# vqdang/hover_net

Measured on AMD Instinct MI355X. Metric: tiles/sec (270x270, batch 32) end-to-end incl. watershed, higher is better.
Workload: dtype fp32

## Files before the change

hover_net_amd/csrc/hvn_api.hip:

```cpp
#include <hip/hip_runtime.h>
#include <stdio.h>
#include <string.h>

#include <vector>

#include "../../include/hvn.h"
#include "hvn_kernels.h"

static thread_local char g_err[512] = "";

static int fail(int code, const char *fmt, const char *a = "", long b = 0)
{
    snprintf(g_err, sizeof(g_err), fmt, a, b);
    return code;
}

extern "C" {

int hvn_version(void) { return 104; }

#ifndef HVN_BUILD_ID
#define HVN_BUILD_ID "unstamped"
#endif
static const char hvn_build_tag[] = "hvn-build-id:" HVN_BUILD_ID;
// ... 48 lines not shown

int hvn_profile_conv_ms_list(double *out, int cap)
{
    if (g_ev_used < 2) return 0;
    hipEventSynchronize(g_ev[g_ev_used - 1]);
    int n = 0;
    for (size_t i = 0; i + 1 < g_ev_used && n < cap; i += 2, ++n) {
        float ms = 0.f;
        hipEventElapsedTime(&ms, g_ev[i], g_ev[i + 1]);
        out[n] = ms;
    }
    return n;
}

static bool aligned16(const void *p) { return (((uintptr_t)p) & 15) == 0; }

static int run_one(const hvn_op *op, int batch, hipStream_t s)
{
    switch (op->kind) {
    case HVN_OP_CONV0: {
        Conv0Args a;
        a.img = op->x.base;
        a.isn = op->x.sn; a.isy = op->x.sy; a.isx = op->x.sx; a.isc = op->x.sc ? op->x.sc : 1;
        a.is_f32 = op->x_dtype;
        a.H = op->x.h; a.W = op->x.w;
        a.w = op->w; a.bias = op->bias;
        a.y = (float *)op->y.base;
        a.ysn = op->y.sn; a.ysy = op->y.sy; a.ysx = op->y.sx;
        a.N = batch; a.Ho = op->y.h; a.Wo = op->y.w; a.pad = op->pad_t; a.relu = op->relu; a.out_bf16 = op->act_dtype == 1;
        if (op->kh != 7 || op->kw != 7 || op->x.c != 3 || op->y.c != 64 || !op->w || !op->bias)
            return fail(HVN_E_ARG, "conv0: expects 7x7x3->64 with bias%s", "");
        if (!aligned16(a.y) || (a.ysx & 3) || (a.ysy & 3) || (a.ysn & 3)) return fail(HVN_E_ARG, "conv0: output view not 16-byte aligned%s", "");
        return hvn_launch_conv0(a, s);
    }
    case HVN_OP_CONV: {
        ConvArgs a;
        memset(&a, 0, sizeof(a));
        a.x = (const float *)op->x.base;
        a.xsn = op->x.sn; a.xsy = op->x.sy; a.xsx = op->x.sx;
        a.H = op->x.h; a.W = op->x.w; a.Cin = op->x.c;
        a.w = op->w; a.bias = op->bias;
        a.pre_s = op->pre_scale; a.pre_b = op->pre_shift;
        a.post_s = op->post_scale; a.post_b = op->post_shift;
        a.res = (const float *)op->res.base;
        a.rsn = op->res.sn; a.rsy = op->res.sy; a.rsx = op->res.sx;
        a.y = (float *)op->y.base;
        a.ysn = op->y.sn; a.ysy = op->y.sy; a.ysx = op->y.sx;
        a.N = batch; a.Ho = op->y.h; a.Wo = op->y.w; a.Cout = op->cout;
        a.KH = op->kh; a.KW = op->kw; a.stride = op->stride; a.pad_t = op->pad_t; a.pad_l = op->pad_l;
        a.relu = op->relu;
        a.groups = op->groups > 1 ? op->groups : 1;
        a.x2 = (const float *)op->x2.base;
        a.x2sn = op->x2.sn; a.x2sy = op->x2.sy; a.x2sx = op->x2.sx;
        a.Cin2 = a.x2 ? op->x2.c : 0;
        a.stride2 = op->_rsv > 0 ? op->_rsv : 1;
        if (a.x2 && (op->kh != 1 || op->kw != 1 || a.stride != 1 || a.Cin2 % 32 || !aligned16(a.x2) || ((a.x2sn | a.x2sy | a.x2sx) & 3) ||
                     a.pre_s || (long)(a.Ho - 1) * a.stride2 >= op->x2.h || (long)(a.Wo - 1) * a.stride2 >= op->x2.w))
            return fail(HVN_E_ARG, "conv: second input needs a 1x1 stride-1 op without prologue and a view that covers the output grid%s", "");
        a.M = (long)batch * a.Ho * a.Wo;
        if (!a.x || !a.w || !a.y) return fail(HVN_E_ARG, "conv: null pointer%s", "");
        if (a.Cin % 32) return fail(HVN_E_ARG, "conv: input channels must be a multiple of 32 (got %s%ld)", "", a.Cin);
        if (!aligned16(a.x) || !aligned16(a.w) || (a.xsx & 3) || (a.xsy & 3) || (a.xsn & 3))
            return fail(HVN_E_ARG, "conv: input view / weights not 16-byte aligned%s", "");
        if ((a.pre_s && !aligned16(a.pre_s)) || (a.pre_b && !aligned16(a.pre_b)) || (!a.pre_s != !a.pre_b))
            return fail(HVN_E_ARG, "conv: prologue vectors must be 16-byte aligned and come in pairs%s", "");
        if (!a.post_s != !a.post_b) return fail(HVN_E_ARG, "conv: epilogue affine must come in pairs%s", "");
        if (op->y.c != op->cout) return fail(HVN_E_ARG, "conv: output view channels != cout%s", "");
        a.nbatch = op->nbatch > 1 ? op->nbatch : 1;
        a.xb = op->batch_stride[0]; a.wb = op->batch_stride[1]; a.yb = op->batch_stride[2];
        if (a.nbatch > 1 && ((a.xb | a.wb | a.yb) & 3)) return fail(HVN_E_ARG, "conv: batch strides must keep 16-byte alignment%s", "");
        const bool bf16 = op->act_dtype == 1;
        if (bf16 && (((a.xsx | a.xsy | a.xsn) & 7) || (a.x2 && ((a.x2sx | a.x2sy | a.x2sn) & 7)) || a.nbatch > 1))
            return fail(HVN_E_ARG, "conv(bf16): input strides must be multiples of 8 elements; no batched launch%s", "");
        if (g_prof) prof_mark(s);
        const bool x3 = op->act_dtype == 2 || op->act_dtype == 3;
        if (x3 && (a.groups > 1 || (a.nbatch > 1 && (a.wb & 7)))) return fail(HVN_E_ARG, "conv(bf16x3): no grouped convs; batch stride of the planes must keep 16-byte alignment%s", "");
        int rc;
        if (bf16 && (op->tile_n == 896 || op->tile_n == 640))
            rc = hvn_launch_conv_bf16g(a, op->tile_n == 896 ? 256 : 128, s);
        else if (bf16)
            rc = hvn_launch_conv_bf16(a, op->tile_n, s);
        else if (x3 && (op->tile_n == 896 || op->tile_n == 640))
            rc = hvn_launch_conv_x3g(a, op->tile_n == 896 ? 256 : 128, op->act_dtype == 3 ? 6 : 9, s);
        else
            rc = x3 ? hvn_launch_conv_x3(a, op->tile_n, op->act_dtype == 3 ? 6 : 9, s) : hvn_launch_conv(a, op->tile_n, s);
        if (g_prof) prof_mark(s);
        if (rc) return fail(rc == -1 ? HVN_E_ARG : HVN_E_LAUNCH, "conv: launch failed (tile_n=%s%ld)", "", op->tile_n);
        return 0;
    }
    case HVN_OP_CHAIN: {
        ChainArgs a;
        memset(&a, 0, sizeof(a));
        a.x = (const float *)op->x.base;
        a.xsn = op->x.sn; a.xsy = op->x.sy; a.xsx = op->x.sx; a.K1 = op->x.c;
        a.x2 = (const float *)op->x2.base;
        a.x2sn = op->x2.sn; a.x2sy = op->x2.sy; a.x2sx = op->x2.sx;
        a.K1b = a.x2 ? op->x2.c : 0;
        a.stride2 = op->_rsv > 0 ? op->_rsv : 1;
        a.w1 = op->w;
        a.res = (const float *)op->res.base;
        a.rsn = op->res.sn; a.rsy = op->res.sy; a.rsx = op->res.sx;
        a.y = (float *)op->y.base;
        a.ysn = op->y.sn; a.ysy = op->y.sy; a.ysx = op->y.sx; a.C = op->cout;
        a.post_s = op->post_scale; a.post_b = op->post_shift;
        a.pre_s = op->pre_scale; a.pre_b = op->pre_shift;
        a.w2 = op->w2; a.bias2 = op->bias2; a.relu2 = 1;
        a.y2 = (float *)op->y2.base;
        a.y2sn = op->y2.sn; a.y2sy = op->y2.sy; a.y2sx = op->y2.sx; a.N2 = op->cout2;
        a.N = batch; a.Ho = op->y.h; a.Wo = op->y.w;
        a.M = (long)batch * a.Ho * a.Wo;
        a.bm = op->tile_n == 64 ? 64 : 128;
        const bool cx3 = op->act_dtype == 2 || op->act_dtype == 3;
        const bool cbf = op->act_dtype == 1;
        if (op->act_dtype != 0 && !cx3 && !cbf) return fail(HVN_E_ARG, "chain: act_dtype 0 (fp32), 1 (bf16) or 2 | 3 (fp32 with bf16x3 products)%s", "");
        if (cbf) {
            if (!a.x || !a.w1 || !a.y || !a.w2 || !a.y2) return fail(HVN_E_ARG, "chain: null pointer%s", "");
            if (op->kh != 1 || op->kw != 1 || op->stride != 1 || op->pad_t || op->pad_l || op->relu || op->bias)
                return fail(HVN_E_ARG, "chain: the first conv is a plain 1x1 (no bias / relu of its own)%s", "");
            if (!hvn_chain_bf16_supported(a.K1, a.K1b, a.C, a.N2) || op->y.c != a.C || op->y2.c != a.N2)
                return fail(HVN_E_ARG, "chain (bf16): needs input channels in slabs of 64 (64 or 128 in all), cout %% 256 == 0, cout2 in {64, 128} (cout2 = %s%ld)", "", a.N2);
            if (op->x.h != a.Ho || op->x.w != a.Wo || op->y2.h != a.Ho || op->y2.w != a.Wo ||
                (a.x2 && ((long)(a.Ho - 1) * a.stride2 >= op->x2.h || (long)(a.Wo - 1) * a.stride2 >= op->x2.w)))
                return fail(HVN_E_ARG, "chain: views do not cover the output grid%s", "");
            if (a.res && (a.rsn != a.ysn || a.rsy != a.ysy || a.rsx != a.ysx || op->res.c != a.C))
                return fail(HVN_E_ARG, "chain: the residual view must have the output's strides%s", "");
            if (!aligned16(a.x) || !aligned16(a.w1) || !aligned16(a.w2) || !aligned16(a.y) || !aligned16(a.y2) || (a.res && !aligned16(a.res)) ||
                (a.x2 && !aligned16(a.x2)) || ((a.xsn | a.xsy | a.xsx | a.ysn | a.ysy | a.ysx | a.y2sn | a.y2sy | a.y2sx | a.x2sn | a.x2sy | a.x2sx) & 7))
                return fail(HVN_E_ARG, "chain (bf16): views / weights not 16-byte aligned%s", "");
            if ((!a.pre_s != !a.pre_b) || (!a.post_s != !a.post_b) || (a.pre_s && (!aligned16(a.pre_s) || !aligned16(a.pre_b))) ||
                (a.post_s && (!aligned16(a.post_s) || !aligned16(a.post_b))) || (a.bias2 && !aligned16(a.bias2)))
                return fail(HVN_E_ARG, "chain: per-channel vectors must be 16-byte aligned and come in pairs%s", "");
            if (g_prof) prof_mark(s);
            const int rcb = hvn_launch_conv_chain_bf16(a, s);
            if (g_prof) prof_mark(s);
            if (rcb) return fail(rcb == -1 ? HVN_E_ARG : HVN_E_LAUNCH, "chain (bf16): launch failed (cout2=%s%ld)", "", a.N2);
            return 0;
        }
        if (!a.x || !a.w1 || !a.y || !a.w2 || !a.y2) return fail(HVN_E_ARG, "chain: null pointer%s", "");
        if (op->kh != 1 || op->kw != 1 || op->stride != 1 || op->pad_t || op->pad_l || op->relu || op->bias)
            return fail(HVN_E_ARG, "chain: the first conv is a plain 1x1 (no bias / relu of its own)%s", "");
        if (!hvn_chain_supported(a.C, a.N2) || op->y.c != a.C || op->y2.c != a.N2 || a.K1 % 32 || a.K1b % 32 || a.K1 + a.K1b < 64)
            return fail(HVN_E_ARG, "chain: needs cout %% 64 == 0, cout2 in {64, 128}, input channels in slabs of 32 (>= 64) (cout2 = %s%ld)", "", a.N2);
        if (op->x.h != a.Ho || op->x.w != a.Wo || op->y2.h != a.Ho || op->y2.w != a.Wo ||
            (a.x2 && ((long)(a.Ho - 1) * a.stride2 >= op->x2.h || (long)(a.Wo - 1) * a.stride2 >= op->x2.w)))
            return fail(HVN_E_ARG, "chain: views do not cover the output grid%s", "");
        if (a.res && (a.rsn != a.ysn || a.rsy != a.ysy || a.rsx != a.ysx || op->res.c != a.C))
            return fail(HVN_E_ARG, "chain: the residual view must have the output's strides%s", "");
        if (!aligned16(a.x) || !aligned16(a.w1) || !aligned16(a.w2) || !aligned16(a.y) || !aligned16(a.y2) || (a.res && !aligned16(a.res)) ||
            (a.x2 && !aligned16(a.x2)) || ((a.xsn | a.xsy | a.xsx | a.ysn | a.ysy | a.ysx | a.y2sn | a.y2sy | a.y2sx | a.x2sn | a.x2sy | a.x2sx) & 3))
            return fail(HVN_E_ARG, "chain: views / weights not 16-byte aligned%s", "");
        if ((!a.pre_s != !a.pre_b) || (!a.post_s != !a.post_b) || (a.pre_s && (!aligned16(a.pre_s) || !aligned16(a.pre_b))) ||
            (a.post_s && (!aligned16(a.post_s) || !aligned16(a.post_b))) || (a.bias2 && !aligned16(a.bias2)))
            return fail(HVN_E_ARG, "chain: per-channel vectors must be 16-byte aligned and come in pairs%s", "");
        if (g_prof) prof_mark(s);
        int rc;
        if (cx3 && op->tile_n == 1152)
            rc = hvn_launch_conv_chain_x3r(a, op->act_dtype == 3 ? 6 : 9, s);
        else
            rc = cx3 ? hvn_launch_conv_chain_x3(a, op->act_dtype == 3 ? 6 : 9, s) : hvn_launch_conv_chain(a, s);
        if (g_prof) prof_mark(s);
        if (rc) return fail(rc == -1 ? HVN_E_ARG : HVN_E_LAUNCH, "chain: launch failed (cout2=%s%ld)", "", a.N2);
        return 0;
    }
    case HVN_OP_WINO_IN:
    case HVN_OP_WINO_OUT: {
        WinoArgs a;
// ... 118 lines not shown
```

hover_net_amd/csrc/hvn_kernels.h:

```cpp
#pragma once
#include <hip/hip_runtime.h>
#include <stdint.h>

#include <atomic>

static inline int hvn_max_lds_once(const void *kern, int bytes, std::atomic<unsigned long long> &done)
{
    int dev = 0;
    if (hipGetDevice(&dev) != hipSuccess) return -2;
    const unsigned long long bit = 1ull << (dev & 63);
    if (done.load(std::memory_order_acquire) & bit) return 0;
    if (hipFuncSetAttribute(kern, hipFuncAttributeMaxDynamicSharedMemorySize, bytes) != hipSuccess) return -2;
    done.fetch_or(bit, std::memory_order_release);
    return 0;
}

struct ConvArgs {
    const float *x;
    long xsn, xsy, xsx;
    int H, W, Cin;
    const float *w;
    const float *bias, *pre_s, *pre_b, *post_s, *post_b;
    const float *res;
    long rsn, rsy, rsx;
    float *y;
    long ysn, ysy, ysx;
    int N, Ho, Wo, Cout, KH, KW, stride, pad_t, pad_l, relu;
    long M;
    long m_tiles;
    int n_tiles;
    int groups;
    const float *x2;
    long x2sn, x2sy, x2sx;
    int Cin2, stride2;
    int nbatch;
    unsigned long long *dbg;
    long xb, wb, yb;
};

int hvn_launch_conv(const ConvArgs &a, int tile_n, hipStream_t stream);

#ifndef HVN_CONV_XCD_CONTIG
#define HVN_CONV_XCD_CONTIG 1
#endif
static __device__ __forceinline__ int hvn_m_tile(int xcd, int seq_m, int groups, bool contiguous)
{
    return (HVN_CONV_XCD_CONTIG && contiguous) ? xcd * groups + seq_m : seq_m * 8 + xcd;
}

struct ChainArgs {
    const float *x;
    long xsn, xsy, xsx;
    int K1;
    const float *x2;
    long x2sn, x2sy, x2sx;
    int K1b, stride2;
    const float *w1;
    const float *res;
    long rsn, rsy, rsx;
    float *y;
    long ysn, ysy, ysx;
    int C;
    const float *post_s, *post_b, *pre_s, *pre_b;
    const float *w2;
    const float *bias2;
    int relu2;
    float *y2;
    long y2sn, y2sy, y2sx;
    int N2;
    int N, Ho, Wo;
    long M;
    int bm;
    unsigned long long *dbg;
};
int hvn_launch_conv_chain(const ChainArgs &a, hipStream_t stream);
int hvn_chain_supported(int c, int n2);
int hvn_chain_bf16_supported(int k1, int k1b, int c, int n2);
int hvn_launch_conv_chain_bf16(const ChainArgs &a, hipStream_t stream);
int hvn_launch_conv_chain_x3(const ChainArgs &a, int terms, hipStream_t stream);
int hvn_chain_x3r_supported(const ChainArgs &a);
int hvn_launch_conv_chain_x3r(const ChainArgs &a, int terms, hipStream_t stream);
int hvn_launch_conv_bf16(const ConvArgs &a, int tile_n, hipStream_t stream);
int hvn_launch_conv_bf16g(const ConvArgs &a, int bm, hipStream_t stream);
int hvn_launch_conv_x3(const ConvArgs &a, int tile_n, int terms, hipStream_t stream);
int hvn_launch_conv_x3g(const ConvArgs &a, int bm, int terms, hipStream_t stream);
int hvn_conv_x3g_supported(const ConvArgs &a, int bm);
int hvn_launch_split_x3(const float *src, uint16_t *dst, long granules, hipStream_t stream);

struct Conv0Args {
    const void *img;
    long isn, isy, isx, isc;
    int is_f32;
    int H, W;
    const float *w;
    const float *bias;
    float *y;
    long ysn, ysy, ysx;
    int N, Ho, Wo, pad;
    int relu;
    int out_bf16;
};
int hvn_launch_conv0(const Conv0Args &a, hipStream_t stream);

struct UpAddArgs {
    const float *lo;
    long lsn, lsy, lsx;
    const float *skip;
    long ssn, ssy, ssx;
    float *y;
    long ysn, ysy, ysx;
    int N, H, W, C;
    int bf16;
};
int hvn_launch_upadd(const UpAddArgs &a, hipStream_t stream);

struct HeadArgs {
    const float *x;
    long xsn, xsy, xsx;
    const float *w;
    const float *bias;
    float *y;
    int N, H, W, Cout;
    int in_bf16;
};
int hvn_launch_head(const HeadArgs &a, hipStream_t stream);

int hvn_launch_extract_patches(const uint8_t *img, int H, int W, const int32_t *coords, int P, int win, int pad_t, int pad_l, uint8_t *out,
                               hipStream_t stream);

struct PredMapArgs {
    const float *tp, *np, *hv;
    float *y;
    int N, H, W, nr_types;
};
int hvn_launch_predmap(const PredMapArgs &a, hipStream_t stream);

struct WinoArgs {
    const float *x;
    long xsn, xsy, xsx;
    float *y;
    long ysn, ysy, ysx;
    const float *mat;
    const float *bias;
    int N, H, W, C;
    int ty, tx, pad, relu;
    int m;
    int r;
    int accum;
    const float *lo;
    long lsn, lsy, lsx;
};
int hvn_launch_wino_in(const WinoArgs &a, hipStream_t stream);
int hvn_launch_wino_out(const WinoArgs &a, hipStream_t stream);

struct PackArgs {
    const float *src;
    float *dst;
    int cout, cin_g, groups, taps;
    int mode;
    int lead_pad;
    const float *gmat;
};
int hvn_launch_pack_w(const PackArgs &a, hipStream_t stream);
int hvn_launch_pack_w_multi(const PackArgs *tbl, const int *first_block, int n, long blocks, hipStream_t stream);

struct WgradArgs {
    const float *x;
    long xsn, xsy, xsx;
    int H, W, Cin;
// ... 114 lines not shown
```

hover_net_amd/engine.py:

```python
import ctypes

import numpy as np
import torch

from . import lib as L
from . import plan as PL


def _view_struct(v, base_ptr, sn, itemsize=4):
    b = v.buf
    sx = b.c
    sy = b.w * b.c
    s = L.hvn_view()
    s.base = base_ptr + (v.y0 * sy + v.x0 * sx + v.c0) * itemsize
    s.sn, s.sy, s.sx = sn, sy, sx
    s.h, s.w, s.c, s.sc = v.h, v.w, v.c, 1
    return s


WG_SLOTS = 512
WG_SLOTS_NARROW = 768
NARROW_TILE_COST = 0.45


def pick_tile_n(op, batch):
    import math
    import os

    if op.tile_n != 128 or os.environ.get("HVN_TILE_SELECT", "auto") == "0":
        return op.tile_n
    force = os.environ.get("HVN_FORCE_TILE_N")
    if force:
        return int(force)
    slots64 = int(os.environ.get("HVN_WG_SLOTS_64", WG_SLOTS_NARROW))
    cost64 = float(os.environ.get("HVN_NARROW_COST", NARROW_TILE_COST))
    m_tiles = math.ceil(batch * op.y.h * op.y.w / 128.0)
    nb = int(op.extra.get("nbatch", 1))
    wide = math.ceil(m_tiles * math.ceil(op.cout / 128.0) * nb / WG_SLOTS)
    narrow = math.ceil(m_tiles * math.ceil(op.cout / 64.0) * nb / slots64) * cost64
    return 64 if narrow < wide else 128


_STREAM_POOL, _STREAM_CHOICE = {}, {}


def lane_stream_pool(device, count):
    have = _STREAM_POOL.setdefault(str(device), [])
    while len(have) < count:
        have.append(torch.cuda.Stream(device))
    return have


_TILE_CACHE = {}
X3G_256, X3G_128 = 128 + 0x300, 128 + 0x200
X3R = 128 + 0x400


def x3g_forms_for(op):
    import os

    want = os.environ.get("HVN_X3G", "1")
    if want == "0" or op.cout < 128 or int(op.extra.get("groups", 1)) != 1:
        return ()
    cin = op.x.c
    forms = []
    for code, bm, na in ((X3G_256, 256, 3), (X3G_128, 128, 2)):
        if want not in ("1", str(code)):
            continue
        if op.pre is not None and bm == 256 and na * bm * 128 + 2 * 3 * 128 * 64 + 2 * cin * 4 > 160 * 1024:
            continue
        forms.append(code)
    return tuple(forms)


def to_bf16_bits(a):
    u = np.ascontiguousarray(a, np.float32).view(np.uint32)
    return ((u + (((u >> 16) & 1) + 0x7FFF)) >> 16).astype(np.uint16)


def repack_conv_bf16(w32):
    cp, s32, taps, _ = w32.shape
    if s32 % 2:
        w32 = np.concatenate([w32, np.zeros((cp, 1, taps, 32), np.float32)], 1)
        s32 += 1
    w = w32.reshape(cp, s32 // 2, 2, taps, 32).transpose(0, 1, 3, 2, 4).reshape(cp, s32 // 2, taps, 64)
    return to_bf16_bits(w)


def split_bf16x3(w32):
    w = np.ascontiguousarray(w32, np.float32)

    def bf(a):
        bits = to_bf16_bits(a)
        return bits, (bits.astype(np.uint32) << 16).view(np.float32)

    h, hf = bf(w)
    r = w - hf
    m, mf = bf(r)
    l, _ = bf(r - mf)
    return h, m, l


def pack_conv_x3(w32):
    lead = w32.shape[:-3]
    kt = w32.shape[-3] * w32.shape[-2]
    planes = split_bf16x3(w32.reshape(lead + (kt, 32)))
    return np.stack(planes, axis=-2)


def pack_conv_x3_device(w32, device):
    w = torch.from_numpy(np.ascontiguousarray(w32, np.float32).reshape(-1, 32)).to(device)
    h = w.to(torch.bfloat16)
    r = w - h.float()
    m = r.to(torch.bfloat16)
    l = (r - m.float()).to(torch.bfloat16)
    return torch.stack((h, m, l), dim=1).view(torch.int16).reshape(-1)


class Engine:
    def __init__(self, plan, max_batch=32, device="cuda", n_split=None, dtype="fp32", n_lanes=None):
        L.require_gpu()
        assert dtype in ("fp32", "bf16")
        self.dtype = dtype
        self.isz = 4 if dtype == "fp32" else 2
        if dtype == "bf16" and any(op.kind in (PL.OP_WINO_IN, PL.OP_WINO_OUT) for op in plan.ops):
            raise ValueError("the bf16 path runs direct convolutions: build the plan with winograd=0")
        self.plan = plan
        self.max_batch = int(max_batch)
        self.device = torch.device(device)
        import os
        dflt = ("2", "2") if dtype == "fp32" else ("1", "0")
        self.n_split = int(os.environ.get("HVN_SPLIT", dflt[0])) if n_split is None else int(n_split)
        self.n_lane_streams = int(os.environ.get("HVN_LANES", dflt[1])) if n_lanes is None else int(n_lanes)
        self.split_decoder = os.environ.get("HVN_SPLIT_DECODER", "0") != "0"
        self._streams = None
        self._stream_off = 0
        self._upload_params()
        self.arena = torch.empty((self.max_batch, plan.arena_per_sample), dtype=torch.float32 if dtype == "fp32" else torch.int16,
                                 device=self.device)
        self.logits = {br: torch.empty((self.max_batch, b.c, b.h, b.w), dtype=torch.float32, device=self.device)
                       for br, b in plan.logits.items()}
        self.pred_map = None
        if plan.pred_map is not None:
            pm = plan.pred_map
            self.pred_map = torch.empty((self.max_batch, pm.h, pm.w, pm.c), dtype=torch.float32, device=self.device)
        self.ops = (L.hvn_op * len(plan.ops))()
        self._bind()
        self._sub_ops = {}
        self.tile_choice = _TILE_CACHE.setdefault(str(self.device), {})
        tile_file = os.environ.get("HVN_TILE_FILE")
        if tile_file and dtype == "fp32":
            import json
            tiles = json.load(open(tile_file))
            if len(tiles) != len(self.ops):
                raise ValueError("HVN_TILE_FILE holds %d entries for a plan of %d ops" % (len(tiles), len(self.ops)))
            for o, op, tn in zip(self.ops, plan.ops, tiles):
                if op.kind == PL.OP_CONV and ((op.tile_n == 128 and (tn in (64, 128) or (op.extra.get("x3") and tn in x3g_forms_for(op)))) or
                                              (op.tile_n == 64 and tn in (64, 320) and not op.extra.get("x3"))):
                    o.tile_n = tn
                if op.kind == PL.OP_CHAIN and (tn in (64, 128) or (tn == X3R and op.extra.get("x3"))):
                    o.tile_n = tn
        elif dtype == "fp32" and os.environ.get("HVN_TILE_SELECT", "auto") == "auto" and not os.environ.get("HVN_FORCE_TILE_N"):
            self.autotune_tiles()
        elif dtype == "bf16" and os.environ.get("HVN_TILE_SELECT", "auto") == "auto" and os.environ.get("HVN_BF16G", "1") != "0":
            self.autotune_bf16_forms()
        if os.environ.get("HVN_TILE_SELECT", "auto") == "auto" and os.environ.get("HVN_STREAM_SELECT", "1") != "0":
            self.autotune_streams()

    def _upload_params(self):
        arrays, offs, total = [], {}, 0

        def put(key, a):
            nonlocal total
            if a is None:
                return
            a = np.ascontiguousarray(a, np.float32).ravel()
            offs[key] = total
            arrays.append((total, a))
            total += (a.size + 63) // 64 * 64

        w16, off16, tot16 = [], {}, 0
        for i, op in enumerate(self.plan.ops):
            if self.dtype == "bf16" and op.kind in (PL.OP_CONV, PL.OP_CHAIN):
                wb = repack_conv_bf16(op.w).ravel()
                off16[i] = tot16
                w16.append((tot16, wb))
                tot16 += (wb.size + 127) // 128 * 128
                if op.kind == PL.OP_CHAIN:
                    wb2 = repack_conv_bf16(op.extra["w2"]).ravel()
                    off16[(i, "w2")] = tot16
                    w16.append((tot16, wb2))
                    tot16 += (wb2.size + 127) // 128 * 128
            elif self.dtype == "fp32" and op.kind in (PL.OP_CONV, PL.OP_CHAIN) and op.extra.get("x3"):
                off16[i] = tot16
                w16.append((tot16, op.w, True))
                tot16 += (3 * op.w.size + 127) // 128 * 128
                if op.kind == PL.OP_CHAIN:
                    off16[(i, "w2")] = tot16
                    w16.append((tot16, op.extra["w2"], True))
                    tot16 += (3 * op.extra["w2"].size + 127) // 128 * 128
            else:
                put((i, "w"), op.w)
            put((i, "bias"), op.bias)
            if not (op.kind == PL.OP_CHAIN and (self.dtype == "bf16" or op.extra.get("x3"))):
                put((i, "w2"), op.extra.get("w2"))
            put((i, "bias2"), op.extra.get("bias2"))
            if op.pre is not None:
                put((i, "pre_s"), op.pre[0])
                put((i, "pre_b"), op.pre[1])
            if op.post is not None:
                put((i, "post_s"), op.post[0])
                put((i, "post_b"), op.post[1])
        host = np.zeros(max(total, 64), np.float32)
        for off, a in arrays:
            host[off:off + a.size] = a
        self.params = torch.from_numpy(host).to(self.device)
        self._poff = offs
        self._poff16 = off16
        self.params16 = None
        if tot16:
            if any(len(e) == 3 for e in w16):
                self.params16 = torch.zeros(tot16, dtype=torch.int16, device=self.device)
                for off, w32, _ in w16:
                    pl = pack_conv_x3_device(w32, self.device)
                    self.params16[off:off + pl.numel()] = pl
            else:
                h16 = np.zeros(tot16, np.uint16)
                for off, a in w16:
                    h16[off:off + a.size] = a
                self.params16 = torch.from_numpy(h16.view(np.int16)).to(self.device)

    def _pptr(self, i, name):
        off = self._poff.get((i, name))
        return None if off is None else self.params.data_ptr() + 4 * off

    def _bind(self):
        P = self.plan
        abase = self.arena.data_ptr()
        sn = P.arena_per_sample
        for i, op in enumerate(P.ops):
            o = self.ops[i]
# ... 67 lines not shown
            for off in range(4):
                self._stream_off, self._streams = off, None
                best = float("inf")
                for r in range(reps + 1):
                    e0.record()
                    self.run(imgs)
                    self.run(imgs)
                    e1.record()
                    e1.synchronize()
                    if r:
                        best = min(best, e0.elapsed_time(e1) / 2)
                ms[off] = best
            _STREAM_CHOICE[key] = (min(ms, key=ms.get), ms)
        self._stream_off, self._streams = _STREAM_CHOICE[key][0], None

    def autotune_tiles(self, reps=3, margin=0.985):
        import os

        lib = L.lib()
        reps = max(1, int(os.environ.get("HVN_TUNE_REPS", reps)))
        stream = torch.cuda.current_stream(self.device).cuda_stream
        e0, e1 = torch.cuda.Event(enable_timing=True), torch.cuda.Event(enable_timing=True)
        osz = ctypes.sizeof(L.hvn_op)
        base = ctypes.addressof(self.ops)

        lanes = getattr(self.plan, "lanes", None)
        enc_end = lanes[0][2] if (lanes and lanes[0][0] == "main" and len(lanes) > 1) else 0
        split = self.n_split if (self.n_split > 1 and self.max_batch >= 2 * self.n_split) else 1
        sub_n = -(-self.max_batch // split)
        if os.environ.get("HVN_TUNE_SUB", "1") == "0":
            sub_n = self.max_batch

        def time_op(i):
            best = float("inf")
            nb = sub_n if (i < enc_end or self.split_decoder) else self.max_batch
            for r in range(reps + 1):
                e0.record()
                L.check(lib.hvn_run_op(base + i * osz, nb, ctypes.c_void_p(stream)), "hvn_run_op (autotune)")
                e1.record()
                e1.synchronize()
                if r:
                    best = min(best, e0.elapsed_time(e1))
            return best

        for i, op in enumerate(self.plan.ops):
            if op.kind == PL.OP_CHAIN and op.extra.get("x3"):
                mode = os.environ.get("HVN_CHAIN_X3R", "1")
                x2 = op.extra.get("x2")
                if mode == "0" or op.x.c != 64 or (x2 is not None and (x2.c != 64 or op.res is not None or op.extra["cout2"] != 64)):
                    continue
                key = ("chain_x3", sub_n if (i < enc_end or self.split_decoder) else self.max_batch, op.x.c, x2.c if x2 is not None else 0, op.cout, op.extra["cout2"],
                       op.y.h, op.y.w, op.res is not None, op.post is not None, op.pre is not None, int(op.extra.get("x3", 0)), mode)
                if key not in self.tile_choice:
                    o = self.ops[i]
                    t = {}
                    for tn in ((X3R,) if mode == "force" else (128, X3R)):
                        o.tile_n = tn
                        t[tn] = time_op(i)
                    best = X3R if (mode == "force" or t[X3R] < margin * t[128]) else 128
                    self.tile_choice[key] = (best, t.get(128, float("nan")), t[X3R], dict(t))
                self.ops[i].tile_n = self.tile_choice[key][0]
                continue
            if op.kind == PL.OP_CHAIN:
                if os.environ.get("HVN_CHAIN_BM"):
                    self.ops[i].tile_n = int(os.environ["HVN_CHAIN_BM"])
                    continue
                x2 = op.extra.get("x2")
                key = ("chain", sub_n if (i < enc_end or self.split_decoder) else self.max_batch, op.x.c, x2.c if x2 is not None else 0, op.cout, op.extra["cout2"], op.y.h, op.y.w, op.res is not None,
                       op.post is not None, op.pre is not None)
                if key not in self.tile_choice:
                    o = self.ops[i]
                    t = {}
                    for tn in (128, 64):
                        o.tile_n = tn
                        t[tn] = time_op(i)
                    self.tile_choice[key] = (64 if t[64] < margin * t[128] else 128, t[128], t[64])
                self.ops[i].tile_n = self.tile_choice[key][0]
                continue
            if op.kind != PL.OP_CONV or op.tile_n not in (128, 64) or int(op.extra.get("groups", 1)) != 1:
                continue
            x2 = op.extra.get("x2")
            key = (sub_n if (i < enc_end or self.split_decoder) else self.max_batch, op.kh, op.kw, op.stride, op.x.c, op.cout, op.y.h, op.y.w, op.x.h, op.x.w, op.res is not None, op.pre is not None,
                   op.post is not None, int(op.extra.get("nbatch", 1)), x2.c if x2 is not None else 0)
            if op.tile_n == 64 and (x2 is not None or op.extra.get("x3")):
                continue
            key = key + (int(op.extra.get("x3", 0)),)
            cands = (128, 64) if op.tile_n == 128 else (64, 320)
            if op.tile_n == 128 and op.extra.get("x3") and x3g_forms_for(op):
                forced = os.environ.get("HVN_X3G_FORCE")
                if forced and int(forced) in x3g_forms_for(op):
                    self.ops[i].tile_n = int(forced)
                    try:
                        time_op(i)
                        continue
                    except L.HvnError:
                        self.ops[i].tile_n = 128
                cands = cands + x3g_forms_for(op)
            key = key + (cands,)
            if key not in self.tile_choice:
                o = self.ops[i]
                t = {}
                for tn in cands:
                    o.tile_n = tn
                    try:
                        t[tn] = time_op(i)
                    except L.HvnError:
                        if tn in (128, 64, 320):
                            raise
                        t[tn] = float("inf")
                best = min(cands[1:], key=lambda tn: t[tn])
                self.tile_choice[key] = (best if t[best] < margin * t[cands[0]] else cands[0], t[cands[0]], t[best], dict(t))
            self.ops[i].tile_n = self.tile_choice[key][0]
        torch.cuda.synchronize(self.device)

    def autotune_bf16_forms(self, reps=3, margin=0.985):
        import os

        lib = L.lib()
        reps = max(1, int(os.environ.get("HVN_TUNE_REPS", reps)))
        stream = torch.cuda.current_stream(self.device).cuda_stream
        e0, e1 = torch.cuda.Event(enable_timing=True), torch.cuda.Event(enable_timing=True)
        osz = ctypes.sizeof(L.hvn_op)
        base = ctypes.addressof(self.ops)
        forced = os.environ.get("HVN_BF16G_FORCE")

        def time_op(i):
            best = float("inf")
            for r in range(reps + 1):
                e0.record()
                L.check(lib.hvn_run_op(base + i * osz, self.max_batch, ctypes.c_void_p(stream)), "hvn_run_op (autotune)")
                e1.record()
                e1.synchronize()
                if r:
                    best = min(best, e0.elapsed_time(e1))
            return best

        for i, op in enumerate(self.plan.ops):
            if op.kind != PL.OP_CONV or self.ops[i].tile_n != 128 or op.pre is not None or op.cout < 128 or int(op.extra.get("nbatch", 1)) > 1:
                continue
            x2 = op.extra.get("x2")
            key = ("bf16", self.max_batch, op.kh, op.kw, op.stride, op.x.c, op.cout, op.y.h, op.y.w, op.x.h, op.x.w, op.res is not None,
                   op.post is not None, x2.c if x2 is not None else 0, int(op.extra.get("groups", 1)))
            key = key + (forced,)
            if key not in self.tile_choice:
                t = {}
                for tn in ((int(forced),) if forced else (128, X3G_256, X3G_128)):
                    self.ops[i].tile_n = tn
                    try:
                        t[tn] = time_op(i)
                    except L.HvnError:
                        if tn == 128:
                            raise
                        t[tn] = float("inf")
                best = min(t, key=t.get)
                if t[best] == float("inf") or (not forced and best != 128 and t[best] >= margin * t[128]):
                    best = 128
                self.tile_choice[key] = (best, t.get(128, float("nan")), t[best], dict(t))
            self.ops[i].tile_n = self.tile_choice[key][0]
        torch.cuda.synchronize(self.device)

    def _set_input(self, imgs):
        o = self.ops[0]
        assert self.plan.ops[0].kind == PL.OP_CONV0
        n = imgs.shape[0]
        if n > self.max_batch:
            raise ValueError("batch %d exceeds the engine's max_batch %d" % (n, self.max_batch))
        g = self.plan.geo["inp"]
        if imgs.dtype == torch.uint8:
            if tuple(imgs.shape[1:]) != (g, g, 3):
                raise ValueError("expected uint8 [N,%d,%d,3] patches, got %s" % (g, g, tuple(imgs.shape)))
# ... 141 lines not shown
```

hover_net_amd/lib.py:

```python
import ctypes
import os
import subprocess

_HERE = os.path.dirname(os.path.abspath(__file__))
LIB_PATH = os.path.join(_HERE, "libhvn_hip.so")
VARIANTS = {
    "pad": ("-DHVN_SWZ=0",),
    "noxcd": ("-DHVN_WINO_XCD=0", "-DHVN_CONV_XCD_CONTIG=0"),
    "fullepi": ("-DHVN_X3G_FULL_EPI=1",),
    "wn1": ("-DHVN_X3G_WN=1",),
    "prev": (),
    "trace": ("-DHVN_TRACE_FINE=1",),
}
CSRC = os.path.join(_HERE, "csrc")
SOURCES = ("hvn_conv.hip", "hvn_conv_chain.hip", "hvn_conv_chain_x3.hip", "hvn_conv_chain_x3r.hip", "hvn_conv_bf16.hip", "hvn_conv_bf16g.hip", "hvn_conv_chain_bf16.hip", "hvn_conv_x3.hip", "hvn_conv_x3g.hip", "hvn_net_ops.hip", "hvn_postproc.hip", "hvn_api.hip", "hvn_train.hip", "hvn_wgrad_x3.hip", "hvn_targets.hip", "hvn_wsi_merge.hip",
           "hvn_augment.hip", "hvn_train_api.hip", "hvn_contour.cpp", "hvn_metrics.hip")
HIPCC_FLAGS = ("--offload-arch=gfx950", "-O3", "-std=c++17", "-fPIC", "-shared", "-ffp-contract=off",
               "-fvisibility=hidden", "-Wno-unused-value", "-pthread")


class hvn_view(ctypes.Structure):
    _fields_ = [("base", ctypes.c_void_p), ("sn", ctypes.c_int64), ("sy", ctypes.c_int64), ("sx", ctypes.c_int64),
                ("h", ctypes.c_int32), ("w", ctypes.c_int32), ("c", ctypes.c_int32), ("sc", ctypes.c_int32)]


class hvn_op(ctypes.Structure):
    _fields_ = [(k, ctypes.c_int32) for k in ("kind", "kh", "kw", "stride", "pad_t", "pad_l", "relu", "cout", "tile_n", "x_dtype", "groups", "_rsv")] + \
               [("x", hvn_view), ("res", hvn_view), ("y", hvn_view), ("x2", hvn_view)] + \
               [(k, ctypes.c_void_p) for k in ("w", "bias", "pre_scale", "pre_shift", "post_scale", "post_shift")] + \
               [("batch_stride", ctypes.c_int64 * 3), ("nbatch", ctypes.c_int32), ("act_dtype", ctypes.c_int32)] + \
               [("y2", hvn_view), ("w2", ctypes.c_void_p), ("bias2", ctypes.c_void_p), ("cout2", ctypes.c_int32), ("_rsv2", ctypes.c_int32)]


class hvn_top(ctypes.Structure):
    _fields_ = [(k, ctypes.c_int32) for k in ("kind", "kh", "kw", "stride", "pad_t", "pad_l", "groups", "cout", "cin_g", "mode", "lead_pad", "_pad")] + \
               [("x", hvn_view), ("y", hvn_view), ("dx", hvn_view), ("dy", hvn_view), ("p", ctypes.c_void_p * 6),
                ("eps", ctypes.c_float), ("momentum", ctypes.c_float), ("net", ctypes.POINTER(hvn_op)),
                ("batch_stride", ctypes.c_int64 * 3), ("nbatch", ctypes.c_int32), ("_pad2", ctypes.c_int32)]


class hvn_pack_desc(ctypes.Structure):
    _fields_ = [("src", ctypes.c_void_p), ("dst", ctypes.c_void_p)] + [(k, ctypes.c_int32) for k in ("cout", "cin_g", "groups", "taps", "mode", "lead_pad")] + \
               [("gmat", ctypes.c_void_p)]


class hvn_loss(ctypes.Structure):
    _fields_ = [(k, ctypes.c_void_p) for k in ("logits_np", "logits_hv", "logits_tp", "true_np", "true_tp", "true_hv",
                                               "grad_np", "grad_hv", "grad_tp", "sums", "sobel_ws")] + \
               [(k, ctypes.c_int32) for k in ("n", "h", "w", "nr_types")] + [("total_pixels", ctypes.c_double), ("weight", ctypes.c_float * 6),
                                                                             ("partials", ctypes.c_void_p), ("partials_cap", ctypes.c_int64)]


class hvn_inst_rec(ctypes.Structure):
    _fields_ = [("label", ctypes.c_int32), ("area", ctypes.c_int32), ("rmin", ctypes.c_int32), ("rmax", ctypes.c_int32),
                ("cmin", ctypes.c_int32), ("cmax", ctypes.c_int32), ("sum_x", ctypes.c_double), ("sum_y", ctypes.c_double),
                ("type", ctypes.c_int32), ("type_count", ctypes.c_int32)]


EXPORTS = (
    "hvn_version", "hvn_build_id", "hvn_last_error", "hvn_device_ok", "hvn_run_plan", "hvn_run_op", "hvn_profile_enable",
    "hvn_profile_conv_ms", "hvn_profile_conv_launches", "hvn_profile_conv_ms_list", "hvn_postproc_workspace_bytes", "hvn_postproc",
    "hvn_postproc_taps", "hvn_postproc_stats", "hvn_instance_table_workspace_bytes", "hvn_instance_table", "hvn_trace_contours",
    "hvn_run_train_plan", "hvn_run_train_plan_ws", "hvn_train_workspace_bytes", "hvn_train_last_error", "hvn_loss_partials_count", "hvn_loss_forward", "hvn_loss_backward", "hvn_adam_step",
    "hvn_extract_patches", "hvn_gen_targets", "hvn_gen_targets_workspace_bytes", "hvn_augment_shape", "hvn_augment_input",
    "hvn_wsi_merge_normal", "hvn_wsi_merge_fixing",
    "hvn_pair_table_workspace_bytes", "hvn_pair_table", "hvn_label_range", "hvn_remap_label_workspace_bytes", "hvn_remap_label",
    "hvn_label_areas", "hvn_label_permute",
)


class HvnError(RuntimeError):
    pass


def source_id():
    import hashlib

    h = hashlib.sha256()
    for f in sorted(SOURCES) + ["hvn_conv_common.h", "hvn_kernels.h"]:
        h.update(f.encode())
        h.update(open(os.path.join(CSRC, f), "rb").read())
    h.update(open(os.path.join(os.path.dirname(_HERE), "include", "hvn.h"), "rb").read())
    h.update(" ".join(HIPCC_FLAGS).encode())
    return h.hexdigest()[:16]


def _built_id(path):
    if not os.path.exists(path):
        return None
    data = open(path, "rb").read()
    i = data.find(b"hvn-build-id:")
    if i < 0:
        return None
    j = data.find(b"\0", i)
    return data[i + 13:j].decode(errors="replace")


_HIPCC_VERSION = None
# ... 164 lines not shown
```

Before: 755.6.

## Add spatial-patch x3 bf16 implicit-GEMM kernel for narrow 3x3 convs

Adds a new x3 (three-way bf16 split) 3x3 stride-1 convolution kernel for convs with Cin 32/64 and Cout up to 64. It loads an 8x16 output patch plus halo into LDS once and reuses it across all nine taps, so the input is not re-gathered per tap. The autotuner now times this form against the existing tile 64 for eligible x3 ops and keeps the faster one. The cost is a new code path with heavy unrolling and a larger LDS footprint.

```diff
diff --git a/hover_net_amd/csrc/hvn_api.hip b/hover_net_amd/csrc/hvn_api.hip
--- a/hover_net_amd/csrc/hvn_api.hip
+++ b/hover_net_amd/csrc/hvn_api.hip
@@ -154,6 +154,8 @@
             rc = hvn_launch_conv_bf16(a, op->tile_n, s);
         else if (x3 && (op->tile_n == 896 || op->tile_n == 640))
             rc = hvn_launch_conv_x3g(a, op->tile_n == 896 ? 256 : 128, op->act_dtype == 3 ? 6 : 9, s);
+        else if (x3 && op->tile_n == 576)
+            rc = hvn_launch_conv_x3p(a, op->act_dtype == 3 ? 6 : 9, s);
         else
             rc = x3 ? hvn_launch_conv_x3(a, op->tile_n, op->act_dtype == 3 ? 6 : 9, s) : hvn_launch_conv(a, op->tile_n, s);
         if (g_prof) prof_mark(s);
diff --git a/hover_net_amd/csrc/hvn_conv_x3p.hip b/hover_net_amd/csrc/hvn_conv_x3p.hip
--- /dev/null
+++ b/hover_net_amd/csrc/hvn_conv_x3p.hip
@@ -0,0 +1,257 @@
+#include <hip/hip_runtime.h>
+#include <stdint.h>
+
+#include <type_traits>
+
+#include "hvn_conv_common.h"
+
+#define XK 32
+#define XPITCH 104
+#define PT_H 8
+#define PT_W 16
+#define PP_W (PT_W + 2)
+#define PP_N ((PT_H + 2) * (PT_W + 2))
+#define EP_LD 68
+
+static __device__ __forceinline__ uint32_t pack2(__bf16 a, __bf16 b)
+{
+    bf16x2 v = {a, b};
+    return __builtin_bit_cast(uint32_t, v);
+}
+
+static __device__ __forceinline__ int x3p_col(int r) { return r < 16 ? r : ((r + 14) & 15); }
+
+template <int NSLAB, int NTERMS>
+__global__ __launch_bounds__(256, 2) void hvn_conv_igemm_x3p(ConvArgs p)
+{
+    static_assert(NTERMS == 9 || NTERMS == 6, "nine exact partial products, or the six that carry > 2^-24 of the product");
+    constexpr int KT = 9 * NSLAB;
+    constexpr int ROWS = PP_N * NSLAB;
+    constexpr int NPASS = (ROWS + 31) / 32;
+    constexpr int NLOAD = NPASS;
+    extern __shared__ __attribute__((aligned(16))) uint16_t xs[];
+
+    const int tid = threadIdx.x;
+    const int lane = tid & 63, wave = tid >> 6;
+    const int l31 = lane & 31, lh = lane >> 5;
+    const int wm = wave >> 1, wn = wave & 1;
+
+    const int xcd = blockIdx.x & 7, seq = blockIdx.x >> 3;
+    const int m_tile = hvn_m_tile(xcd, seq, (int)(gridDim.x >> 3), true);
+    if (m_tile >= (int)p.m_tiles) return;
+    const int tiles_x = (p.Wo + PT_W - 1) / PT_W, tiles_y = (p.Ho + PT_H - 1) / PT_H;
+    const int n = m_tile / (tiles_x * tiles_y);
+    const int t = m_tile - n * (tiles_x * tiles_y);
+    const int oy0 = (t / tiles_x) * PT_H, ox0 = (t % tiles_x) * PT_W;
+
+    {
+        const __amdgpu_buffer_rsrc_t rsrc_a = hvn_buf(p.x + (long)n * p.xsn);
+        const int srow = tid >> 3, scol = (tid & 7) * 4;
+#pragma unroll
+        for (int b = 0; b < NPASS / NLOAD; ++b) {
+            f32x4 ra[NLOAD];
+#pragma unroll
+            for (int j = 0; j < NLOAD; ++j) {
+                const int row = srow + 32 * (b * NLOAD + j);
+                const int px = row / NSLAB, slab = row - px * NSLAB;
+                const int py = px / PP_W;
+                const int iy = oy0 + py - p.pad_t, ix = ox0 + (px - py * PP_W) - p.pad_l;
+                const bool ok = row < ROWS && (unsigned)iy < (unsigned)p.H && (unsigned)ix < (unsigned)p.W;
+                const unsigned vo = ok ? (unsigned)(((long)iy * p.xsy + (long)ix * p.xsx + slab * XK + scol) * 4) : HVN_OOB;
+                ra[j] = hvn_buf_load16(rsrc_a, vo, 0);
+            }
+#pragma unroll
+            for (int j = 0; j < NLOAD; ++j) {
+                const int row = srow + 32 * (b * NLOAD + j);
+                const int px = row / NSLAB, slab = row - px * NSLAB;
+                const f32x4 v = ra[j];
+                __bf16 h[4], m[4], l[4];
+                hvn_split3(v.x, h[0], m[0], l[0]);
+                hvn_split3(v.y, h[1], m[1], l[1]);
+                hvn_split3(v.z, h[2], m[2], l[2]);
+                hvn_split3(v.w, h[3], m[3], l[3]);
+                if (row < ROWS) {
+                    uint16_t *dst = xs + (slab * PP_N + px) * XPITCH + scol;
+                    *(u32x2 *)(dst) = (u32x2){pack2(h[0], h[1]), pack2(h[2], h[3])};
+                    *(u32x2 *)(dst + 32) = (u32x2){pack2(m[0], m[1]), pack2(m[2], m[3])};
+                    *(u32x2 *)(dst + 64) = (u32x2){pack2(l[0], l[1]), pack2(l[2], l[3])};
+                }
+            }
+        }
+    }
+
+    const __amdgpu_buffer_rsrc_t rsrc_w = hvn_buf(p.w);
+    const int brow = wn * 32 + l31;
+    const unsigned w_voff = brow < p.Cout ? (unsigned)(brow * (KT * 192) + lh * 16) : HVN_OOB;
+    u32x4 fbr[2][3][2];
+    auto load_b = [&](int kt, int st) {
+#pragma unroll
+        for (int pl = 0; pl < 3; ++pl)
+#pragma unroll
+            for (int q = 0; q < 2; ++q) fbr[st][pl][q] = __builtin_amdgcn_raw_buffer_load_b128(rsrc_w, w_voff, kt * 192 + pl * 64 + q * 32, 0);
+    };
+    load_b(0, 0);
+
+    f32x16 acc[2];
+#pragma unroll
+    for (int i = 0; i < 2; ++i)
+#pragma unroll
+        for (int r = 0; r < 16; ++r) acc[i][r] = 0.f;
+
+    const uint16_t *a0 = xs + ((4 * wm + (l31 >> 4)) * PP_W + x3p_col(l31)) * XPITCH + 8 * lh;
+    u32x4 far[2][2][3];
+    auto load_a = [&](int hs, int st) {
+        const int kt = hs >> 1, q = hs & 1;
+        const int slab = kt / 9, tr = (kt % 9) / 3, ts = kt % 3;
+        const uint16_t *a = a0 + (slab * PP_N + tr * PP_W + ts) * XPITCH + q * 16;
+#pragma unroll
+        for (int i = 0; i < 2; ++i)
+#pragma unroll
+            for (int pl = 0; pl < 3; ++pl) far[st][i][pl] = *(const u32x4 *)(a + i * 2 * PP_W * XPITCH + pl * 32);
+    };
+
+    __syncthreads();
+
+    load_a(0, 0);
+    __builtin_amdgcn_sched_barrier(0);
+#pragma unroll
+    for (int hs = 0; hs < 2 * KT; ++hs) {
+        const int kt = hs >> 1, q = hs & 1;
+        if (q == 0 && kt + 1 < KT) load_b(kt + 1, (kt + 1) & 1);
+        if (hs + 1 < 2 * KT) load_a(hs + 1, (hs + 1) & 1);
+        __builtin_amdgcn_sched_barrier(0);
+#pragma unroll
+        for (int s = 4; s >= 0; --s) {
+            if (NTERMS == 6 && s > 2) continue;
+#pragma unroll
+            for (int pa = 2; pa >= 0; --pa) {
+                const int pb = s - pa;
+                if (pb < 0 || pb > 2) continue;
+#pragma unroll
+                for (int i = 0; i < 2; ++i)
+                    acc[i] = __builtin_amdgcn_mfma_f32_32x32x16_bf16(__builtin_bit_cast(bf16x8, far[hs & 1][i][pa]), __builtin_bit_cast(bf16x8, fbr[kt & 1][pb][q]),
+                                                                     acc[i], 0, 0, 0);
+            }
+        }
+        __builtin_amdgcn_sched_barrier(0);
+    }
+    __syncthreads();
+
+    float *ep = (float *)xs;
+#pragma unroll
+    for (int i = 0; i < 2; ++i)
+#pragma unroll
+        for (int r = 0; r < 16; ++r) {
+            const int mr = (r & 3) + 8 * (r >> 2) + 4 * lh;
+            const int row = (4 * wm + 2 * i + (mr >> 4)) * PT_W + x3p_col(mr);
+            ep[row * EP_LD + wn * 32 + l31] = acc[i][r];
+        }
+    __syncthreads();
+    constexpr int NIT = PT_H;
+    const int ecol = (tid & 15) * 4;
+    const int etx = tid >> 4;
+    const int co = ecol;
+    const bool cok = co < p.Cout;
+    f32x4 bias = {0.f, 0.f, 0.f, 0.f}, qs = {1.f, 1.f, 1.f, 1.f}, qb = bias;
+    const bool has_res = p.res != nullptr, has_post = p.post_s != nullptr;
+    if (cok) {
+        if (p.bias) bias = *(const f32x4 *)(p.bias + co);
+        if (has_post) {
+            qs = *(const f32x4 *)(p.post_s + co);
+            qb = *(const f32x4 *)(p.post_b + co);
+        }
+    }
+    const float relu_lo = p.relu ? 0.f : -__builtin_inff();
+    const float post_lo = has_post ? 0.f : -__builtin_inff();
+    const bool xok = cok && ox0 + etx < p.Wo;
+    unsigned y_off = (unsigned)(((long)oy0 * p.ysy + (long)(ox0 + etx) * p.ysx + co) * 4);
+    unsigned r_off = (unsigned)(((long)oy0 * p.rsy + (long)(ox0 + etx) * p.rsx + co) * 4);
+    const unsigned y_step = (unsigned)(p.ysy * 4), r_step = (unsigned)(p.rsy * 4);
+    const __amdgpu_buffer_rsrc_t rsrc_y = hvn_buf(p.y + (long)n * p.ysn);
+    const __amdgpu_buffer_rsrc_t rsrc_r = hvn_buf(has_res ? p.res + (long)n * p.rsn : p.y + (long)n * p.ysn);
+    f32x4 rall[NIT], vout[NIT];
+    unsigned yoffs[NIT];
+#pragma unroll
+    for (int it = 0; it < NIT; ++it) {
+        const bool ok = xok && oy0 + it < p.Ho;
+        rall[it] = (f32x4){0.f, 0.f, 0.f, 0.f};
+        if (has_res) rall[it] = hvn_buf_load16(rsrc_r, ok ? r_off : HVN_OOB, 0);
+        yoffs[it] = ok ? y_off : HVN_OOB;
+        y_off += y_step;
+        r_off += r_step;
+    }
+    auto finish = [&](auto hb_t, auto hr_t, auto hp_t) {
+        constexpr bool HB = decltype(hb_t)::value, HR = decltype(hr_t)::value, HP = decltype(hp_t)::value;
+#pragma unroll
+        for (int it = 0; it < NIT; ++it) {
+            f32x4 v = *(const f32x4 *)(ep + (it * PT_W + etx) * EP_LD + ecol);
+            if constexpr (HB) {
+                v.x = fmaxf(v.x + bias.x, relu_lo);
+                v.y = fmaxf(v.y + bias.y, relu_lo);
+                v.z = fmaxf(v.z + bias.z, relu_lo);
+                v.w = fmaxf(v.w + bias.w, relu_lo);
+            }
+            if constexpr (HR) v += rall[it];
+            if constexpr (HP) {
+                v.x = fmaxf(fmaf(v.x, qs.x, qb.x), post_lo);
+                v.y = fmaxf(fmaf(v.y, qs.y, qb.y), post_lo);
+                v.z = fmaxf(fmaf(v.z, qs.z, qb.z), post_lo);
+                v.w = fmaxf(fmaf(v.w, qs.w, qb.w), post_lo);
+            }
+            vout[it] = v;
+        }
+    };
+    {
+        using T = std::true_type;
+        using F = std::false_type;
+        const bool hb = p.bias != nullptr || p.relu;
+        if (hb) {
+            if (has_res) {
+                if (has_post) finish(T{}, T{}, T{}); else finish(T{}, T{}, F{});
+            } else {
+                if (has_post) finish(T{}, F{}, T{}); else finish(T{}, F{}, F{});
+            }
+        } else {
+            if (has_res) {
+                if (has_post) finish(F{}, T{}, T{}); else finish(F{}, T{}, F{});
+            } else {
+                if (has_post) finish(F{}, F{}, T{}); else finish(F{}, F{}, F{});
+            }
+        }
+    }
+#pragma unroll
+    for (int it = 0; it < NIT; ++it) asm volatile("" : "+v"(vout[it]), "+v"(yoffs[it]));
+    __builtin_amdgcn_sched_barrier(0);
+#pragma unroll
+    for (int it = 0; it < NIT; ++it) hvn_buf_store16(vout[it], rsrc_y, yoffs[it], 0);
+}
+
+template <int NSLAB, int NTERMS>
+static int launch_x3p(ConvArgs p, hipStream_t stream)
+{
+    constexpr size_t patch_b = (size_t)NSLAB * PP_N * XPITCH * 2, ep_b = (size_t)PT_H * PT_W * EP_LD * 4;
+    constexpr size_t lds = patch_b > ep_b ? patch_b : ep_b;
+    static std::atomic<unsigned long long> attr_done{0};
+    const long tiles = (long)p.N * ((p.Ho + PT_H - 1) / PT_H) * ((p.Wo + PT_W - 1) / PT_W);
+    const long grid = (tiles + 7) / 8 * 8;
+    if (tiles <= 0 || grid > 0x7fffffffL) return -1;
+    p.m_tiles = tiles;
+    p.n_tiles = 1;
+    if (hvn_max_lds_once((const void *)hvn_conv_igemm_x3p<NSLAB, NTERMS>, (int)lds, attr_done)) return -2;
+    hipLaunchKernelGGL((hvn_conv_igemm_x3p<NSLAB, NTERMS>), dim3((unsigned)grid), dim3(256), lds, stream, p);
+    return hipGetLastError() == hipSuccess ? 0 : -2;
+}
+
+int hvn_launch_conv_x3p(const ConvArgs &a, int terms, hipStream_t stream)
+{
+    if (a.KH != 3 || a.KW != 3 || a.stride != 1 || a.groups > 1 || a.x2 || a.pre_s || a.pre_b || a.nbatch > 1) return -1;
+    if ((a.Cin != 32 && a.Cin != 64) || a.Cout <= 0 || a.Cout > 64 || a.Cout % 4 != 0) return -1;
+    if (a.N <= 0 || a.H <= 0 || a.W <= 0 || a.Ho <= 0 || a.Wo <= 0 || a.pad_t < 0 || a.pad_l < 0) return -1;
+    if (a.M != (long)a.N * a.Ho * a.Wo) return -1;
+    if ((((uintptr_t)a.x | (uintptr_t)a.w | (uintptr_t)a.y | (uintptr_t)a.res | (uintptr_t)a.bias | (uintptr_t)a.post_s | (uintptr_t)a.post_b) & 15) ||
+        ((a.xsn | a.xsy | a.xsx | a.ysn | a.ysy | a.ysx) & 3) || (a.res && ((a.rsn | a.rsy | a.rsx) & 3)))
+        return -1;
+    if (!hvn_conv_reach_ok(a, PT_H * PT_W, 4, 256, false, true)) return -1;
+    if (a.Cin == 64) return terms == 6 ? launch_x3p<2, 6>(a, stream) : launch_x3p<2, 9>(a, stream);
+    return terms == 6 ? launch_x3p<1, 6>(a, stream) : launch_x3p<1, 9>(a, stream);
+}
diff --git a/hover_net_amd/csrc/hvn_kernels.h b/hover_net_amd/csrc/hvn_kernels.h
--- a/hover_net_amd/csrc/hvn_kernels.h
+++ b/hover_net_amd/csrc/hvn_kernels.h
@@ -85,6 +85,7 @@
 int hvn_launch_conv_x3(const ConvArgs &a, int tile_n, int terms, hipStream_t stream);
 int hvn_launch_conv_x3g(const ConvArgs &a, int bm, int terms, hipStream_t stream);
 int hvn_conv_x3g_supported(const ConvArgs &a, int bm);
+int hvn_launch_conv_x3p(const ConvArgs &a, int terms, hipStream_t stream);
 int hvn_launch_split_x3(const float *src, uint16_t *dst, long granules, hipStream_t stream);
 
 struct Conv0Args {
diff --git a/hover_net_amd/engine.py b/hover_net_amd/engine.py
--- a/hover_net_amd/engine.py
+++ b/hover_net_amd/engine.py
@@ -54,6 +54,7 @@
 _TILE_CACHE = {}
 X3G_256, X3G_128 = 128 + 0x300, 128 + 0x200
 X3R = 128 + 0x400
+X3P = 64 + 0x200
 
 
 def x3g_forms_for(op):
@@ -71,6 +72,18 @@
             continue
         forms.append(code)
     return tuple(forms)
+
+
+def x3p_form_for(op):
+    import os
+
+    if os.environ.get("HVN_X3P", "1") == "0" or not op.extra.get("x3") or op.kind != PL.OP_CONV or op.tile_n != 64:
+        return ()
+    if (op.kh, op.kw, op.stride) != (3, 3, 1) or op.x.c not in (32, 64) or op.cout > 64 or int(op.extra.get("groups", 1)) != 1:
+        return ()
+    if op.pre is not None or op.extra.get("x2") is not None or int(op.extra.get("nbatch", 1)) > 1:
+        return ()
+    return (X3P,)
 
 
 def to_bf16_bits(a):
@@ -156,7 +169,8 @@
                 raise ValueError("HVN_TILE_FILE holds %d entries for a plan of %d ops" % (len(tiles), len(self.ops)))
             for o, op, tn in zip(self.ops, plan.ops, tiles):
                 if op.kind == PL.OP_CONV and ((op.tile_n == 128 and (tn in (64, 128) or (op.extra.get("x3") and tn in x3g_forms_for(op)))) or
-                                              (op.tile_n == 64 and tn in (64, 320) and not op.extra.get("x3"))):
+                                              (op.tile_n == 64 and tn in (64, 320) and not op.extra.get("x3")) or
+                                              (op.tile_n == 64 and tn in (64,) + x3p_form_for(op))):
                     o.tile_n = tn
                 if op.kind == PL.OP_CHAIN and (tn in (64, 128) or (tn == X3R and op.extra.get("x3"))):
                     o.tile_n = tn
@@ -390,10 +404,16 @@
             x2 = op.extra.get("x2")
             key = (sub_n if (i < enc_end or self.split_decoder) else self.max_batch, op.kh, op.kw, op.stride, op.x.c, op.cout, op.y.h, op.y.w, op.x.h, op.x.w, op.res is not None, op.pre is not None,
                    op.post is not None, int(op.extra.get("nbatch", 1)), x2.c if x2 is not None else 0)
-            if op.tile_n == 64 and (x2 is not None or op.extra.get("x3")):
+            if op.tile_n == 64 and (x2 is not None or op.extra.get("x3")) and not x3p_form_for(op):
                 continue
             key = key + (int(op.extra.get("x3", 0)),)
             cands = (128, 64) if op.tile_n == 128 else (64, 320)
+            if op.tile_n == 64 and op.extra.get("x3"):
+                if os.environ.get("HVN_X3P_FORCE", "0") not in ("", "0"):
+                    self.ops[i].tile_n = X3P
+                    time_op(i)
+                    continue
+                cands = (64,) + x3p_form_for(op)
             if op.tile_n == 128 and op.extra.get("x3") and x3g_forms_for(op):
                 forced = os.environ.get("HVN_X3G_FORCE")
                 if forced and int(forced) in x3g_forms_for(op):
diff --git a/hover_net_amd/lib.py b/hover_net_amd/lib.py
--- a/hover_net_amd/lib.py
+++ b/hover_net_amd/lib.py
@@ -13,7 +13,7 @@
     "trace": ("-DHVN_TRACE_FINE=1",),
 }
 CSRC = os.path.join(_HERE, "csrc")
-SOURCES = ("hvn_conv.hip", "hvn_conv_chain.hip", "hvn_conv_chain_x3.hip", "hvn_conv_chain_x3r.hip", "hvn_conv_bf16.hip", "hvn_conv_bf16g.hip", "hvn_conv_chain_bf16.hip", "hvn_conv_x3.hip", "hvn_conv_x3g.hip", "hvn_net_ops.hip", "hvn_postproc.hip", "hvn_api.hip", "hvn_train.hip", "hvn_wgrad_x3.hip", "hvn_targets.hip", "hvn_wsi_merge.hip",
+SOURCES = ("hvn_conv.hip", "hvn_conv_chain.hip", "hvn_conv_chain_x3.hip", "hvn_conv_chain_x3r.hip", "hvn_conv_bf16.hip", "hvn_conv_bf16g.hip", "hvn_conv_chain_bf16.hip", "hvn_conv_x3.hip", "hvn_conv_x3g.hip", "hvn_conv_x3p.hip", "hvn_net_ops.hip", "hvn_postproc.hip", "hvn_api.hip", "hvn_train.hip", "hvn_wgrad_x3.hip", "hvn_targets.hip", "hvn_wsi_merge.hip",
            "hvn_augment.hip", "hvn_train_api.hip", "hvn_contour.cpp", "hvn_metrics.hip")
 HIPCC_FLAGS = ("--offload-arch=gfx950", "-O3", "-std=c++17", "-fPIC", "-shared", "-ffp-contract=off",
                "-fvisibility=hidden", "-Wno-unused-value", "-pthread")
```

After: 744.4. -1.5%, worse.
